# memcached/memcached

Measured on AMD Instinct MI355X. Metric: CRC32C GiB/s over device-resident item batches; % of HBM roofline, higher is better.
Workload: dtype u8; 1 GPU; BASELINE configs[1]: 1 Mi items x 4096 B per GPU, stride 4096, one 32-lane group per item (K1 k_fixed<slice-by-4, 32 lanes, 8 x 16-B pieces per lane at 512-B spacing, non-temporal coalesced loads, half-item folds in the last-step tables, four items reduced per tree>); items_per_gpu=1048576, item_bytes=4096, parallelism=items sharded across 1 rank(s), no collective on the data path

## Files before the change

memcached_amd/csrc/k_consts.h:

```cpp
#pragma once

#include <stdint.h>

#if defined(__HIPCC__)
#define MCRC_HD __host__ __device__ __forceinline__
#else
#define MCRC_HD static inline
#endif

namespace mcrc_dev {

constexpr uint32_t kK1Bytes = 4096;
constexpr uint32_t kRowBytes = 1024;
constexpr uint32_t kBlockBytes = 4 * kRowBytes;
constexpr uint32_t kSegBytes = 128 * 1024;
constexpr uint32_t kMaxSpan = 0x7fff0000u;
constexpr uint32_t kGridAlign = 128;
constexpr uint32_t kFragMax = 128;
constexpr uint32_t kWholeMax = 512;
MCRC_HD bool frag_drop(uint32_t len, uint64_t g1o, uint64_t vlen) {
    return len != 0 && (g1o <= kFragMax || vlen <= kWholeMax);
}
constexpr uint32_t kLineBytes = 128;
constexpr uint32_t kEpoch = 32;
MCRC_HD bool lines_fused(int64_t lines_bytes) {
    return lines_bytes >= (int64_t)(kBlockBytes - kLineBytes) && lines_bytes <= (int64_t)kBlockBytes;
}
constexpr uint32_t kSmallMax = 8192;
constexpr uint32_t kSpanBlock = 1024;
constexpr uint32_t kPlanThreads = 1024, kPlanPer = 2, kPlanTile = kPlanThreads * kPlanPer;
constexpr uint32_t kWalkWaves = 4;

}
```

memcached_amd/csrc/k_fixed.h:

```cpp
#pragma once

#include "k_common.h"

namespace mcrc_dev {

struct K1Half {
    uint4 d[4];
    uint32_t cin;
};
__device__ __forceinline__ uint32_t k1_half_value(const K1Half &r, const LaneCtx &c) {
    constexpr uint32_t kShift[3] = {kAuxShift0, kAuxShift1, kAuxShift2};
    uint32_t x[4];
#pragma unroll
    for (int k = 0; k < 4; ++k) x[k] = r.d[k].x;
#pragma unroll
    for (int i = 1; i < 4; ++i)
#pragma unroll
        for (int k = 0; k < 4; ++k) x[k] = step4_next(x[k], dw4(r.d[k], i), c);
#pragma unroll
    for (int k = 0; k < 4; ++k) x[k] = k < 3 ? step4_last_shifted(x[k], kShift[k]) : step4_next(x[k], 0u, c);
    return xor3(x[0], x[1], x[2]) ^ x[3];
}

template <bool CRCIN, bool NT>
__global__ __launch_bounds__(1024) void k_fixed(const uint8_t *__restrict__ base, uint64_t stride,
                                                uint64_t nitems, const uint4 *__restrict__ img,
                                                const uint32_t *__restrict__ crc_in,
                                                uint32_t *__restrict__ out) {
    extern __shared__ __attribute__((aligned(16))) char smem[];
    load_tables(smem, img, kLdsImageK1Bytes);
    constexpr uint32_t IPW = 2;
    const uint32_t lane = threadIdx.x & 63u;
    const uint32_t li = lane & 31u;
    const uint32_t g = lane >> 5;
    const LaneCtx c = make_lane_ctx(li);
    const uint64_t waves = blockDim.x >> 6;
    const uint64_t gstep = gridDim.x * waves;
    const uint64_t ngroups = (nitems + IPW - 1) / IPW;
    uint64_t grp = __builtin_amdgcn_readfirstlane(blockIdx.x * (uint32_t)waves + (threadIdx.x >> 6));
    if (gstep % 65521u) grp = (grp * 65521u) % gstep;
    const uint64_t cg = (ngroups + gstep - 1) / gstep;
    const uint64_t gend = min((grp + 1) * cg, ngroups);
    grp *= cg;
    if (grp >= ngroups) return;
    const uint64_t glast = gend - 1;
    auto item_of = [&](uint64_t gi) { return gi * IPW + g; };

    auto ldh = [&](K1Half &r, uint64_t gi, int q) {
        const bool real = gi < gend;
        const uint64_t gu = real ? gi : glast;
        const uint64_t first = gu * IPW;
        const uint8_t *wb = real ? base + first * stride : reinterpret_cast<const uint8_t *>(img);
        const uint32_t gl = first + g < nitems ? g : (uint32_t)(nitems - 1 - first);
        if (q == 0) {
            if constexpr (CRCIN) r.cin = crc_in[first + gl];
            else r.cin = 0u;
        }
        const uint32_t loff = (real ? gl * (uint32_t)stride : g * kK1Bytes) + li * kK1LaneBytes + 4u * kK1Piece * (uint32_t)q;
#pragma unroll
        for (int k = 0; k < 4; ++k)
            r.d[k] = NT ? ld16_nt(wb + loff + k * kK1Piece) : ld16((gbyte *)(wb + loff + k * kK1Piece));
        __builtin_amdgcn_sched_barrier(0);
    };
    auto half0 = [&](K1Half &m) {
        if (li == 0) m.d[0].x ^= ~m.cin;
        return apply_op<4>(kAuxSpanFold, k1_half_value(m, c));
    };
    auto part0 = [&](uint32_t u0, K1Half &m1) {
        return reduce_level<0>(u0 ^ k1_half_value(m1, c), (lane & 1u) == 0u);
    };
    K1Half h0, h1, h2, h3;
    const uint64_t nsteps = gend - grp;
    ldh(h0, grp, 0);
    ldh(h1, grp, 1);
    ldh(h2, grp + 1, 0);
    auto step_even = [&](uint64_t s) {
        ldh(h3, s + 1, 1);
        const uint32_t u0 = half0(h0);
        ldh(h0, s + 2, 0);
        return part0(u0, h1);
    };
    auto step_odd = [&](uint64_t s) {
        ldh(h1, s + 1, 1);
        const uint32_t u0 = half0(h2);
        ldh(h2, s + 2, 0);
        return part0(u0, h3);
    };
    uint64_t k = 0;
    for (; k + 4 <= nsteps; k += 4) {
        const uint32_t va = step_even(grp);
        const uint32_t vb = step_odd(grp + 1);
        const uint32_t vab = group_pair_level1(va, vb, lane);
        const uint32_t vc = step_even(grp + 2);
        const uint32_t vd = step_odd(grp + 3);
        const uint32_t raw = group_reduce32_quad_span(vab, group_pair_level1(vc, vd, lane), lane);
        const uint64_t item = item_of(grp + (li & 3u));
        if (li < 4 && item < nitems) out[item] = ~raw;
        grp += 4;
    }
    for (; k + 2 <= nsteps; k += 2) {
        const uint32_t va = step_even(grp);
        const uint32_t vb = step_odd(grp + 1);
        const uint32_t raw = group_reduce32_pair_span(va, vb, lane);
        const uint64_t item = item_of(li == 0 ? grp : grp + 1);
        if (li < 2 && item < nitems) out[item] = ~raw;
        grp += 2;
    }
    if (nsteps & 1) {
        const uint32_t raw = group_reduce32_single_span(step_even(grp), lane);
        const uint64_t item = item_of(grp);
        if (li == 0 && item < nitems) out[item] = ~raw;
    }
}

}
```

Measured before the change: 5999 GiB/s.

## Pace K1 waves with workgroup barriers every four-step pass

```diff
diff --git a/memcached_amd/csrc/k_consts.h b/memcached_amd/csrc/k_consts.h
--- a/memcached_amd/csrc/k_consts.h
+++ b/memcached_amd/csrc/k_consts.h
@@ -11,6 +11,10 @@
 namespace mcrc_dev {
 
 constexpr uint32_t kK1Bytes = 4096;
+constexpr uint32_t kK1RoundSteps = 4;
+static_assert(kK1RoundSteps >= 4 && kK1RoundSteps % 4 == 0, "a round is whole passes of K1's 4-step loop");
+constexpr uint32_t kK1RoundsMinSteps = 32;
+MCRC_HD uint64_t k1_rounds(uint64_t cg, uint32_t S) { return cg >= kK1RoundsMinSteps ? cg / S : 0; }
 constexpr uint32_t kRowBytes = 1024;
 constexpr uint32_t kBlockBytes = 4 * kRowBytes;
 constexpr uint32_t kSegBytes = 128 * 1024;
diff --git a/memcached_amd/csrc/k_fixed.h b/memcached_amd/csrc/k_fixed.h
--- a/memcached_amd/csrc/k_fixed.h
+++ b/memcached_amd/csrc/k_fixed.h
@@ -22,19 +22,28 @@
     return xor3(x[0], x[1], x[2]) ^ x[3];
 }
 
-template <bool CRCIN, bool NT>
-__global__ __launch_bounds__(1024) void k_fixed(const uint8_t *__restrict__ base, uint64_t stride,
-                                                uint64_t nitems, const uint4 *__restrict__ img,
-                                                const uint32_t *__restrict__ crc_in,
-                                                uint32_t *__restrict__ out) {
-    extern __shared__ __attribute__((aligned(16))) char smem[];
-    load_tables(smem, img, kLdsImageK1Bytes);
+__device__ __forceinline__ void k1_round_barrier() {
+    __builtin_amdgcn_sched_barrier(0);
+    __builtin_amdgcn_s_barrier();
+    __builtin_amdgcn_sched_barrier(0);
+}
+
+struct K1NoProbe {
+    __device__ __forceinline__ void steps(uint64_t ) const {}
+    __device__ __forceinline__ void exit() const {}
+};
+
+template <bool CRCIN, bool NT, class Probe>
+__device__ __forceinline__ void k_fixed_body(const uint8_t *__restrict__ base, uint64_t stride, uint64_t nitems,
+                                             const uint4 *__restrict__ img, const uint32_t *__restrict__ crc_in,
+                                             uint32_t *__restrict__ out, uint32_t nthreads,
+                                             const Probe &probe) {
     constexpr uint32_t IPW = 2;
     const uint32_t lane = threadIdx.x & 63u;
     const uint32_t li = lane & 31u;
     const uint32_t g = lane >> 5;
     const LaneCtx c = make_lane_ctx(li);
-    const uint64_t waves = blockDim.x >> 6;
+    const uint64_t waves = nthreads >> 6;
     const uint64_t gstep = gridDim.x * waves;
     const uint64_t ngroups = (nitems + IPW - 1) / IPW;
     uint64_t grp = __builtin_amdgcn_readfirstlane(blockIdx.x * (uint32_t)waves + (threadIdx.x >> 6));
@@ -42,7 +51,8 @@
     const uint64_t cg = (ngroups + gstep - 1) / gstep;
     const uint64_t gend = min((grp + 1) * cg, ngroups);
     grp *= cg;
-    if (grp >= ngroups) return;
+    uint64_t owed = k1_rounds(cg, kK1RoundSteps);
+    const bool busy = grp < ngroups;
     const uint64_t glast = gend - 1;
     auto item_of = [&](uint64_t gi) { return gi * IPW + g; };
 
@@ -70,10 +80,6 @@
         return reduce_level<0>(u0 ^ k1_half_value(m1, c), (lane & 1u) == 0u);
     };
     K1Half h0, h1, h2, h3;
-    const uint64_t nsteps = gend - grp;
-    ldh(h0, grp, 0);
-    ldh(h1, grp, 1);
-    ldh(h2, grp + 1, 0);
     auto step_even = [&](uint64_t s) {
         ldh(h3, s + 1, 1);
         const uint32_t u0 = half0(h0);
@@ -86,31 +92,54 @@
         ldh(h2, s + 2, 0);
         return part0(u0, h3);
     };
-    uint64_t k = 0;
-    for (; k + 4 <= nsteps; k += 4) {
-        const uint32_t va = step_even(grp);
-        const uint32_t vb = step_odd(grp + 1);
-        const uint32_t vab = group_pair_level1(va, vb, lane);
-        const uint32_t vc = step_even(grp + 2);
-        const uint32_t vd = step_odd(grp + 3);
-        const uint32_t raw = group_reduce32_quad_span(vab, group_pair_level1(vc, vd, lane), lane);
-        const uint64_t item = item_of(grp + (li & 3u));
-        if (li < 4 && item < nitems) out[item] = ~raw;
-        grp += 4;
+    if (busy) {
+        const uint64_t nsteps = gend - grp;
+        ldh(h0, grp, 0);
+        ldh(h1, grp, 1);
+        ldh(h2, grp + 1, 0);
+        uint64_t k = 0;
+        for (; k + 4 <= nsteps; k += 4) {
+            const uint32_t va = step_even(grp);
+            const uint32_t vb = step_odd(grp + 1);
+            const uint32_t vab = group_pair_level1(va, vb, lane);
+            const uint32_t vc = step_even(grp + 2);
+            const uint32_t vd = step_odd(grp + 3);
+            const uint32_t raw = group_reduce32_quad_span(vab, group_pair_level1(vc, vd, lane), lane);
+            const uint64_t item = item_of(grp + (li & 3u));
+            if (li < 4 && item < nitems) out[item] = ~raw;
+            grp += 4;
+            if ((k + 4) % kK1RoundSteps == 0 && owed) {
+                k1_round_barrier();
+                --owed;
+            }
+            probe.steps(k + 4);
+        }
+        for (; k + 2 <= nsteps; k += 2) {
+            const uint32_t va = step_even(grp);
+            const uint32_t vb = step_odd(grp + 1);
+            const uint32_t raw = group_reduce32_pair_span(va, vb, lane);
+            const uint64_t item = item_of(li == 0 ? grp : grp + 1);
+            if (li < 2 && item < nitems) out[item] = ~raw;
+            grp += 2;
+        }
+        if (nsteps & 1) {
+            const uint32_t raw = group_reduce32_single_span(step_even(grp), lane);
+            const uint64_t item = item_of(grp);
+            if (li == 0 && item < nitems) out[item] = ~raw;
+        }
     }
-    for (; k + 2 <= nsteps; k += 2) {
-        const uint32_t va = step_even(grp);
-        const uint32_t vb = step_odd(grp + 1);
-        const uint32_t raw = group_reduce32_pair_span(va, vb, lane);
-        const uint64_t item = item_of(li == 0 ? grp : grp + 1);
-        if (li < 2 && item < nitems) out[item] = ~raw;
-        grp += 2;
-    }
-    if (nsteps & 1) {
-        const uint32_t raw = group_reduce32_single_span(step_even(grp), lane);
-        const uint64_t item = item_of(grp);
-        if (li == 0 && item < nitems) out[item] = ~raw;
-    }
+    for (; owed; --owed) k1_round_barrier();
+    probe.exit();
+}
+
+template <bool CRCIN, bool NT>
+__global__ __launch_bounds__(1024) void k_fixed(const uint8_t *__restrict__ base, uint64_t stride,
+                                                uint64_t nitems, const uint4 *__restrict__ img,
+                                                const uint32_t *__restrict__ crc_in,
+                                                uint32_t *__restrict__ out) {
+    extern __shared__ __attribute__((aligned(16))) char smem[];
+    load_tables(smem, img, kLdsImageK1Bytes);
+    k_fixed_body<CRCIN, NT>(base, stride, nitems, img, crc_in, out, blockDim.x, K1NoProbe{});
 }
 
 }
```

New measurement: 6240 GiB/s, median of 6. +4.0%, better.
